# naver-ai/egtr

Measured on AMD Instinct MI355X. Metric: images/sec end-to-end SGG, 600x1000 input, N=200 queries, higher is better.
Workload: dtype f32; 1 GPU; VG inference: ResNet-50, N=200, 6 enc/6 dec, 150 classes, 50 predicates, 600x1000, bs=1/GPU fp32 (BASELINE configs[1]); hip_graph=True, gemm_tuning=True, miopen_find=True, parallelism=replicas x1 (independent images, no collective)

## Files before the change

### egtr_amd/csrc/rel_head.hip

```cpp
#include <hip/hip_runtime.h>
#include <stdint.h>

#include "common.h"
#include "xs_format.h"

namespace {

typedef float f32x16 __attribute__((ext_vector_type(16)));

__device__ __forceinline__ f32x16 mfma32(float a, float b, f32x16 c) {
  return __builtin_amdgcn_mfma_f32_32x32x2f32(a, b, c, 0, 0, 0);
}

constexpr int kHd = 256;
constexpr int kH1Stride = 260;

typedef float f32x4v __attribute__((ext_vector_type(4)));

template <int OFF>
__device__ __forceinline__ f32x4v gload_b128(const float4* p) {
  f32x4v v;
  asm volatile("global_load_dwordx4 %0, %1, off offset:%2" : "=&v"(v) : "v"(p), "n"(OFF));
  return v;
}
// ... 471 lines not shown
  float* dst = rel_logits + (size_t)p0 * R;
  for (int pp = 0; pp < npair; ++pp) {
    const int tb = s_tb[pp];
    for (int r = lane; r < R; r += 64) {
      float v = s_out[pp * kStride + r] + b3r[r];
      if (tb >= 0) v += triplet[tb + r];
      dst[(size_t)pp * R + r] = v;
    }
  }
}

constexpr int kHp = 264;

typedef float f32x2v __attribute__((ext_vector_type(2)));
using xs::pack_hi16;
using xs::Split3;

__device__ __forceinline__ f32x4v gload_b128_s(unsigned voff, const void* sbase) {
  f32x4v v;
  asm volatile("global_load_dwordx4 %0, %1, %2" : "=&v"(v) : "v"(voff), "s"(sbase));
  return v;
}
__device__ __forceinline__ f32x4v gload_b128_s1k(unsigned voff, const void* sbase) {
  f32x4v v;
  asm volatile("global_load_dwordx4 %0, %1, %2 offset:1024" : "=&v"(v) : "v"(voff), "s"(sbase));
  return v;
}
__device__ __forceinline__ f32x4v gload_b128_s2k(unsigned voff, const void* sbase) {
  f32x4v v;
  asm volatile("global_load_dwordx4 %0, %1, %2 offset:2048" : "=&v"(v) : "v"(voff), "s"(sbase));
  return v;
}

template <int PRE>
struct PrefetchX6 {
  template <int I>
  static __device__ __forceinline__ void issue(f32x4v (&wq)[PRE][3], unsigned voff, const char* wtile) {
    wq[I][0] = gload_b128_s(voff, wtile + I * 3072);
    wq[I][1] = gload_b128_s1k(voff, wtile + I * 3072);
    wq[I][2] = gload_b128_s2k(voff, wtile + I * 3072);
    if constexpr (I + 1 < PRE) issue<I + 1>(wq, voff, wtile);
  }
  template <int S>
  static __device__ __forceinline__ void run(f32x4v (&wq)[PRE][3], unsigned voff, const char* wtile,
                                             const __bf16* hrow, f32x16& acc_m, f32x16& acc_c) {
    constexpr int newer = 3 * ((15 - S) < (PRE - 1) ? (15 - S) : (PRE - 1));
    vm_wait<newer>(wq[S % PRE][0]);
    vm_wait<newer>(wq[S % PRE][1]);
    vm_wait<newer>(wq[S % PRE][2]);
    const bf16x8 whi = __builtin_bit_cast(bf16x8, wq[S % PRE][0]);
    const bf16x8 wmid = __builtin_bit_cast(bf16x8, wq[S % PRE][1]);
    const bf16x8 wlo = __builtin_bit_cast(bf16x8, wq[S % PRE][2]);
    const bf16x8 hhi = *reinterpret_cast<const bf16x8*>(hrow + 16 * S);
    const bf16x8 hmid = *reinterpret_cast<const bf16x8*>(hrow + 32 * kHp + 16 * S);
    const bf16x8 hlo = *reinterpret_cast<const bf16x8*>(hrow + 64 * kHp + 16 * S);
    acc_c = mfma_bf16(whi, hlo, acc_c);
    acc_m = mfma_bf16(whi, hhi, acc_m);
    acc_c = mfma_bf16(wlo, hhi, acc_c);
    acc_c = mfma_bf16(wmid, hmid, acc_c);
    acc_c = mfma_bf16(whi, hmid, acc_c);
    acc_c = mfma_bf16(wmid, hhi, acc_c);
    if constexpr (S + PRE < 16) {
      wq[S % PRE][0] = gload_b128_s(voff, wtile + (S + PRE) * 3072);
      wq[S % PRE][1] = gload_b128_s1k(voff, wtile + (S + PRE) * 3072);
      wq[S % PRE][2] = gload_b128_s2k(voff, wtile + (S + PRE) * 3072);
    }
    if constexpr (S + 1 < 16) run<S + 1>(wq, voff, wtile, hrow, acc_m, acc_c);
  }
};

template <int PRE>
struct PrefetchX1 {
  template <int I>
  static __device__ __forceinline__ void issue(f32x4v (&wq)[PRE][1], unsigned voff, const char* wtile) {
    wq[I][0] = gload_b128_s(voff, wtile + I * 1024);
    if constexpr (I + 1 < PRE) issue<I + 1>(wq, voff, wtile);
  }
  template <int S>
  static __device__ __forceinline__ void run(f32x4v (&wq)[PRE][1], unsigned voff, const char* wtile,
                                             const __bf16* hrow, f32x16& acc) {
    constexpr int newer = (15 - S) < (PRE - 1) ? (15 - S) : (PRE - 1);
    vm_wait<newer>(wq[S % PRE][0]);
    const bf16x8 w = __builtin_bit_cast(bf16x8, wq[S % PRE][0]);
    const bf16x8 h = *reinterpret_cast<const bf16x8*>(hrow + 16 * S);
    acc = mfma_bf16(w, h, acc);
    if constexpr (S + PRE < 16) wq[S % PRE][0] = gload_b128_s(voff, wtile + (S + PRE) * 1024);
    if constexpr (S + 1 < 16) run<S + 1>(wq, voff, wtile, hrow, acc);
  }
};

template <int T, int OT, bool SAVE = false, int TERMS = 6>
__global__ __launch_bounds__(64 * kRhWaves) __attribute__((amdgpu_waves_per_eu(2, 2))) void rel_head_fwd_x6(
    const float* __restrict__ gate_q, const float* __restrict__ gate_k, const float* __restrict__ uq,
    const float* __restrict__ uk, const float* __restrict__ b1, const unsigned short* __restrict__ w2xr,
    const float* __restrict__ b2r, const unsigned short* __restrict__ w3xr, const float* __restrict__ b3r,
    const unsigned short* __restrict__ w2xc, const float* __restrict__ b2c, const float* __restrict__ w3c,
    const float* __restrict__ b3c, const float* __restrict__ triplet, const int64_t* __restrict__ node_cls, int B,
    int N, int R, int C1, float* __restrict__ rel_logits, float* __restrict__ conn_logits,
    float* __restrict__ gate_mean, int apply_sigmoid, float* __restrict__ h1_save, float* __restrict__ h2_save) {
  static_assert(TERMS == 6 || TERMS == 1, "six exact cross terms or one product of rounded operands");
  constexpr int kPieces = TERMS == 6 ? 3 : 1;
  constexpr int kStride = 32 * OT + 1;
  static_assert(kRhWaves * 32 * kStride * 4 <= kPieces * 32 * kHp * 2, "output tiles fit in the h1 buffer");
  __shared__ __attribute__((aligned(16))) __bf16 s_h[kPieces * 32 * kHp];
  float* const s_out = reinterpret_cast<float*>(s_h);
  __shared__ int s_tb[32];
  __shared__ long long s_pp[32];
  __shared__ float s_cacc[kRhWaves][32];
  constexpr int kH2Pitch = 36;
  __shared__ __attribute__((aligned(16))) float s_h2[SAVE ? kRhWaves * 8 * kH2Pitch : 4];
  const int lane = threadIdx.x & 63, pi = lane & 31, hf = lane >> 5;
  const int wv = __builtin_amdgcn_readfirstlane(threadIdx.x >> 6);
  const int mlp = blockIdx.y;
  const long long total = (long long)B * N * N;
  const int tj = (N + 3) >> 2, ti = (N + 7) >> 3;
  const int b = blockIdx.x / (ti * tj);
  const int trem = blockIdx.x - b * ti * tj;
  const int i0 = (trem / tj) * 8, j0 = (trem - (trem / tj) * tj) * 4;
  const int i_raw = i0 + (pi >> 2), j_raw = j0 + (pi & 3);
  const bool valid = i_raw < N && j_raw < N;
  const int i = i_raw < N ? i_raw : N - 1, j = j_raw < N ? j_raw : N - 1;
  const long long p = ((long long)b * N + i) * N + j;
  const size_t qi = (size_t)b * N + i, kj = (size_t)b * N + j;

  if (SAVE && wv == 0 && hf == 0) s_pp[pi] = valid ? p : -1;
  float g[T];
#pragma unroll
  for (int t = 0; t < T; ++t) {
    const float x = gate_q[qi * T + t] + gate_k[kj * T + t];
    g[t] = 1.f / (1.f + expf(-x));
  }
  if (gate_mean != nullptr && mlp == 0 && wv == 0) {
#pragma unroll
    for (int t = 0; t < T; ++t) {
      float v = (valid && hf == 0) ? g[t] : 0.f;
#pragma unroll
      for (int o = 1; o < 64; o <<= 1) v += __shfl_xor(v, o);
      if (lane == 0) unsafeAtomicAdd(gate_mean + t, v / (float)total);
    }
  }

  {
    const int krow_l = (int)kj;
    const float4 bias4 = reinterpret_cast<const float4*>(b1 + mlp * kHd)[lane];
    const float4* uq4 = reinterpret_cast<const float4*>(uq) + mlp * (kHd / 4) + lane;
    const float4* uk4 = reinterpret_cast<const float4*>(uk) + mlp * (kHd / 4) + lane;
    constexpr int ROW4 = 2 * kHd / 4;
    float4 kk[4][T];
#pragma unroll
    for (int jj = 0; jj < 4; ++jj) {
      const int kr = __builtin_amdgcn_readlane(krow_l, jj);
      const float4* pk = uk4 + (size_t)kr * T * ROW4;
#pragma unroll
      for (int t = 0; t < T; ++t) kk[jj][t] = pk[t * ROW4];
    }
    auto qrow_of = [&](int ii) { return b * N + (i0 + ii < N ? i0 + ii : N - 1); };
    const int ii0 = wv * (8 / kRhWaves);
    float4 ua[2][T];
    {
      const float4* pq = uq4 + (size_t)qrow_of(ii0) * T * ROW4;
#pragma unroll
      for (int t = 0; t < T; ++t) ua[0][t] = pq[t * ROW4];
    }
#pragma unroll
    for (int iu = 0; iu < 8 / kRhWaves; ++iu) {
      const int ii = ii0 + iu;
      if (iu + 1 < 8 / kRhWaves) {
        const float4* pq = uq4 + (size_t)qrow_of(ii + 1) * T * ROW4;
#pragma unroll
        for (int t = 0; t < T; ++t) ua[(iu + 1) & 1][t] = pq[t * ROW4];
      }
#pragma unroll
      for (int jj = 0; jj < 4; ++jj) {
        const int pp = ii * 4 + jj;
        f32x2v a01 = {bias4.x, bias4.y}, a23 = {bias4.z, bias4.w};
#pragma unroll
        for (int t = 0; t < T; ++t) {
          const float4 a = ua[iu & 1][t];
          const float4 c = kk[jj][t];
          const float gt = __int_as_float(__builtin_amdgcn_readlane(__float_as_int(g[t]), pp));
          const f32x2v gg = {gt, gt};
          const f32x2v u01 = {a.x + c.x, a.y + c.y}, u23 = {a.z + c.z, a.w + c.w};
          a01 = gg * u01 + a01;
          a23 = gg * u23 + a23;
        }
        if (SAVE && i0 + ii < N && j0 + jj < N)
          reinterpret_cast<float4*>(h1_save + ((size_t)mlp * total +
                                               (size_t)(((long long)b * N + i0 + ii) * N + j0 + jj)) * kHd)[lane] =
              make_float4(egtr_relu(a01.x), egtr_relu(a01.y), egtr_relu(a23.x), egtr_relu(a23.y));
        if constexpr (TERMS == 1) {
          *reinterpret_cast<uint2*>(s_h + pp * kHp + 4 * lane) =
              make_uint2(xs::cvt_pk_bf16_rne(egtr_relu(a01.x), egtr_relu(a01.y)),
                         xs::cvt_pk_bf16_rne(egtr_relu(a23.x), egtr_relu(a23.y)));
        } else {
          const Split3 sx = xs::split3_fast(egtr_relu(a01.x)), sy = xs::split3_fast(egtr_relu(a01.y)),
                       sz = xs::split3_fast(egtr_relu(a23.x)), sw = xs::split3_fast(egtr_relu(a23.y));
          __bf16* hp = s_h + pp * kHp + 4 * lane;
          *reinterpret_cast<uint2*>(hp) = make_uint2(pack_hi16(sx.hi, sy.hi), pack_hi16(sz.hi, sw.hi));
          *reinterpret_cast<uint2*>(hp + 32 * kHp) = make_uint2(pack_hi16(sx.mid, sy.mid), pack_hi16(sz.mid, sw.mid));
          *reinterpret_cast<uint2*>(hp + 64 * kHp) = make_uint2(pack_hi16(sx.lo, sy.lo), pack_hi16(sz.lo, sw.lo));
        }
      }
    }
    __syncthreads();
  }

  const char* w2x = reinterpret_cast<const char*>(mlp ? w2xc : w2xr);
  const float* b2 = mlp ? b2c : b2r;
  f32x16 racc[OT];
#pragma unroll
  for (int ot = 0; ot < OT; ++ot)
#pragma unroll
    for (int r = 0; r < 16; ++r) racc[ot][r] = 0.f;
  float cacc = 0.f;
  const unsigned voff = (unsigned)lane * 16u;
  const __bf16* hrow = s_h + pi * kHp + 8 * hf;

  constexpr int kNtPerWave = kHd / 32 / kRhWaves;
#pragma unroll 1
  for (int nt = wv * kNtPerWave; nt < (wv + 1) * kNtPerWave; ++nt) {
    f32x16 acc, accc;
#pragma unroll
    for (int r = 0; r < 16; ++r) accc[r] = 0.f;
#pragma unroll
    for (int rq = 0; rq < 4; ++rq) {
      const float4 bb = *reinterpret_cast<const float4*>(b2 + nt * 32 + 8 * rq + 4 * hf);
      acc[4 * rq + 0] = bb.x; acc[4 * rq + 1] = bb.y; acc[4 * rq + 2] = bb.z; acc[4 * rq + 3] = bb.w;
    }
    constexpr int kFrag = kPieces * 1024;
    const char* wtile = w2x + (size_t)nt * (16 * kFrag);
    constexpr int kPre = 4;
    f32x4v wq[kPre][kPieces];
    f32x4v w3q[2 * OT][kPieces];
    if (mlp == 0) {
      const char* w3t = reinterpret_cast<const char*>(w3xr) + (size_t)nt * (2 * OT * kFrag);
#pragma unroll
      for (int f = 0; f < 2 * OT; ++f) {
        w3q[f][0] = gload_b128_s(voff, w3t + f * kFrag);
        if constexpr (TERMS == 6) {
          w3q[f][1] = gload_b128_s1k(voff, w3t + f * kFrag);
          w3q[f][2] = gload_b128_s2k(voff, w3t + f * kFrag);
        }
      }
    }
    if constexpr (TERMS == 1) {
      PrefetchX1<kPre>::template issue<0>(wq, voff, wtile);
      PrefetchX1<kPre>::template run<0>(wq, voff, wtile, hrow, acc);
#pragma unroll
      for (int r = 0; r < 16; ++r) acc[r] = egtr_relu(acc[r]);
    } else {
      PrefetchX6<kPre>::template issue<0>(wq, voff, wtile);
      PrefetchX6<kPre>::template run<0>(wq, voff, wtile, hrow, acc, accc);
#pragma unroll
      for (int r = 0; r < 16; ++r) acc[r] = egtr_relu(acc[r] + accc[r]);
    }
    if (SAVE) {
      float* stg = s_h2 + wv * (8 * kH2Pitch);
#pragma unroll
      for (int i = 0; i < 4; ++i) {
        if ((pi >> 3) == i) {
#pragma unroll
          for (int rq = 0; rq < 4; ++rq)
            *reinterpret_cast<float4*>(stg + (pi & 7) * kH2Pitch + 8 * rq + 4 * hf) =
                make_float4(acc[4 * rq + 0], acc[4 * rq + 1], acc[4 * rq + 2], acc[4 * rq + 3]);
        }
        __builtin_amdgcn_fence(__ATOMIC_RELEASE, "wavefront");
        __builtin_amdgcn_wave_barrier();
        __builtin_amdgcn_fence(__ATOMIC_ACQUIRE, "wavefront");
        const int pr = lane >> 3, ch = lane & 7;
        const float4 v = *reinterpret_cast<const float4*>(stg + pr * kH2Pitch + 4 * ch);
        const long long po = s_pp[8 * i + pr];
        if (po >= 0) *reinterpret_cast<float4*>(h2_save + ((size_t)mlp * total + (size_t)po) * kHd + nt * 32 + 4 * ch) = v;
        __builtin_amdgcn_fence(__ATOMIC_RELEASE, "wavefront");
        __builtin_amdgcn_wave_barrier();
        __builtin_amdgcn_fence(__ATOMIC_ACQUIRE, "wavefront");
      }
    }
    if (mlp == 0) {
#pragma unroll
      for (int f = 0; f < 2 * OT; ++f) {
        if constexpr (TERMS == 1) asm volatile("" : "+v"(w3q[f][0]));
        else asm volatile("" : "+v"(w3q[f][0]), "+v"(w3q[f][1]), "+v"(w3q[f][2]));
      }
#pragma unroll
      for (int kb = 0; kb < 2; ++kb) {
// ... 12 lines not shown
          Split3 sp[8];
#pragma unroll
          for (int e = 0; e < 8; ++e) sp[e] = xs::split3_fast(acc[8 * kb + e]);
          phi = make_uint4(pack_hi16(sp[0].hi, sp[1].hi), pack_hi16(sp[2].hi, sp[3].hi), pack_hi16(sp[4].hi, sp[5].hi),
                           pack_hi16(sp[6].hi, sp[7].hi));
          pmid = make_uint4(pack_hi16(sp[0].mid, sp[1].mid), pack_hi16(sp[2].mid, sp[3].mid),
                            pack_hi16(sp[4].mid, sp[5].mid), pack_hi16(sp[6].mid, sp[7].mid));
          plo = make_uint4(pack_hi16(sp[0].lo, sp[1].lo), pack_hi16(sp[2].lo, sp[3].lo), pack_hi16(sp[4].lo, sp[5].lo),
                           pack_hi16(sp[6].lo, sp[7].lo));
        }
        const bf16x8 hhi = __builtin_bit_cast(bf16x8, phi), hmid = __builtin_bit_cast(bf16x8, pmid),
                     hlo = __builtin_bit_cast(bf16x8, plo);
#pragma unroll
        for (int ot = 0; ot < OT; ++ot) {
          const bf16x8 whi = __builtin_bit_cast(bf16x8, w3q[kb * OT + ot][0]);
          const bf16x8 wmid = __builtin_bit_cast(bf16x8, w3q[kb * OT + ot][1]);
          const bf16x8 wlo = __builtin_bit_cast(bf16x8, w3q[kb * OT + ot][2]);
          racc[ot] = mfma_bf16(whi, hlo, racc[ot]);
          racc[ot] = mfma_bf16(wlo, hhi, racc[ot]);
          racc[ot] = mfma_bf16(wmid, hmid, racc[ot]);
          racc[ot] = mfma_bf16(whi, hmid, racc[ot]);
          racc[ot] = mfma_bf16(wmid, hhi, racc[ot]);
          racc[ot] = mfma_bf16(whi, hhi, racc[ot]);
        }
        }
      }
    } else {
#pragma unroll
      for (int rq = 0; rq < 4; ++rq) {
        const float4 w = *reinterpret_cast<const float4*>(w3c + nt * 32 + 8 * rq + 4 * hf);
        cacc += w.x * acc[4 * rq + 0] + w.y * acc[4 * rq + 1] + w.z * acc[4 * rq + 2] + w.w * acc[4 * rq + 3];
      }
    }
  }

  if (mlp == 1) {
    cacc += __shfl_xor(cacc, 32);
    if (hf == 0) s_cacc[wv][pi] = cacc;
    __syncthreads();
    if (wv == 0 && valid && hf == 0) {
      float v = s_cacc[0][pi];
#pragma unroll
      for (int w = 1; w < kRhWaves; ++w) v += s_cacc[w][pi];
      v += b3c[0];
      conn_logits[p] = apply_sigmoid ? 1.f / (1.f + expf(-v)) : v;
    }
    return;
  }
  __syncthreads();
  float* const my_out = s_out + wv * 32 * kStride;
#pragma unroll
  for (int ot = 0; ot < OT; ++ot)
#pragma unroll
    for (int r = 0; r < 16; ++r) {
      const int ro = ot * 32 + (r & 3) + 8 * (r >> 2) + 4 * hf;
      my_out[pi * kStride + ro] = racc[ot][r];
    }
  if (wv == 0 && hf == 0) {
    int tb = -1;
    if (triplet != nullptr) tb = ((int)node_cls[qi] * C1 + (int)node_cls[kj]) * R;
    s_tb[pi] = tb;
    s_pp[pi] = valid ? p : -1;
  }
  __syncthreads();
  for (int pp = wv; pp < 32; pp += kRhWaves) {
    const long long po = s_pp[pp];
    if (po < 0) continue;
    const int tb = s_tb[pp];
    float* dst = rel_logits + (size_t)po * R;
    for (int r = lane; r < R; r += 64) {
      float v = s_out[pp * kStride + r];
#pragma unroll
      for (int w = 1; w < kRhWaves; ++w) v += s_out[(w * 32 + pp) * kStride + r];
      v += b3r[r];
      if (tb >= 0) v += triplet[tb + r];
      dst[r] = apply_sigmoid ? 1.f / (1.f + expf(-v)) : v;
    }
  }
}

template <int T>
int launch_T(hipStream_t st, int R, dim3 grid, const float* gate_q, const float* gate_k, const float* uq,
             const float* uk, const float* b1, const float* w2r, const float* b2r, const float* w3r,
             const float* b3r, const float* w2c, const float* b2c, const float* w3c, const float* b3c,
             const float* triplet, const int64_t* node_cls, int B, int N, int C1, float* rel, float* conn,
             float* gate_mean, float* h1_save, float* h2_save) {
  if (R <= 32)
    hipLaunchKernelGGL((rel_head_fwd_f32<T, 1>), grid, dim3(64 * kRhWaves), 0, st, gate_q, gate_k, uq, uk, b1, w2r, b2r, w3r,
                       b3r, w2c, b2c, w3c, b3c, triplet, node_cls, B, N, R, C1, rel, conn, gate_mean, h1_save,
                       h2_save);
  else
    hipLaunchKernelGGL((rel_head_fwd_f32<T, 2>), grid, dim3(64 * kRhWaves), 0, st, gate_q, gate_k, uq, uk, b1, w2r, b2r, w3r,
                       b3r, w2c, b2c, w3c, b3c, triplet, node_cls, B, N, R, C1, rel, conn, gate_mean, h1_save,
                       h2_save);
  return 0;
}

template <int T, bool KPASS>
__global__ __launch_bounds__(256) void rel_head_bwd_pairs_f32(
    const float* __restrict__ dh1, const float* __restrict__ gate_q, const float* __restrict__ gate_k,
    const float* __restrict__ utab , int B, int N,
    float* __restrict__ dutab , float* __restrict__ dz ,
    float* __restrict__ dgate_k ) {
  __shared__ float s_g[256 * T];
  __shared__ __attribute__((aligned(16))) float s_red[4 * T * 512];
  __shared__ float s_dk[4 * T];
  const int tid = threadIdx.x, lane = tid & 63, wave = tid >> 6;
  const int b = blockIdx.x / N, f = blockIdx.x - b * N;
  const size_t total = (size_t)B * N * N;
  const float* gfix = (KPASS ? gate_k : gate_q) + ((size_t)b * N + f) * T;
  const float* gvar = (KPASS ? gate_q : gate_k) + (size_t)b * N * T;
// ... 191 lines not shown
    if (num_rel <= 32)                                                                                               \
      hipLaunchKernelGGL((rel_head_fwd_bf16w<TT, 1>), grid, dim3(64), 0, st, gate_q, gate_k, uq, uk, b1, w2r, b2r, w3r, \
                         b3r, w2c, b2c, w3c, b3c, triplet_dist, node_cls, batch, num_query, num_rel, num_cls_plus1,  \
                         rel_logits, conn_logits, gate_mean);                                                        \
    else                                                                                                             \
      hipLaunchKernelGGL((rel_head_fwd_bf16w<TT, 2>), grid, dim3(64), 0, st, gate_q, gate_k, uq, uk, b1, w2r, b2r, w3r, \
                         b3r, w2c, b2c, w3c, b3c, triplet_dist, node_cls, batch, num_query, num_rel, num_cls_plus1,  \
                         rel_logits, conn_logits, gate_mean);                                                        \
    break;
  switch (num_slots) {
    EGTR_TB(1) EGTR_TB(2) EGTR_TB(3) EGTR_TB(4) EGTR_TB(5) EGTR_TB(6) EGTR_TB(7) EGTR_TB(8) EGTR_TB(9) EGTR_TB(10)
    default: return EGTR_E_UNSUPPORTED;
  }
#undef EGTR_TB
  return egtr_check_launch();
}


extern "C" int egtr_rel_head_forward_bf16x6_f32(egtr_stream_t stream, const float* gate_q, const float* gate_k,
                                                const float* uq, const float* uk, const float* b1,
                                                const uint16_t* w2x_rel, const float* b2r, const uint16_t* w3x_rel,
                                                const float* b3r, const uint16_t* w2x_conn, const float* b2c,
                                                const float* w3c, const float* b3c, const float* triplet_dist,
                                                const int64_t* node_cls, int batch, int num_query, int num_slots,
                                                int hidden, int num_rel, int num_cls_plus1, float* rel_logits,
                                                float* conn_logits, float* gate_mean, int apply_sigmoid) {
  if (!gate_q || !gate_k || !uq || !uk || !b1 || !w2x_rel || !b2r || !w3x_rel || !b3r || !w2x_conn || !b2c || !w3c ||
      !b3c || !rel_logits || !conn_logits)
    return EGTR_E_ARG;
  if (triplet_dist != nullptr && node_cls == nullptr) return EGTR_E_ARG;
  if (batch <= 0 || num_query <= 0 || num_slots <= 0 || num_rel <= 0) return EGTR_E_ARG;
  if (hidden != kHd || num_rel > 64 || num_slots > 9) return EGTR_E_UNSUPPORTED;
  hipStream_t st = static_cast<hipStream_t>(stream);
  const long long tiles = (long long)batch * ((num_query + 7) / 8) * ((num_query + 3) / 4);
  if (tiles >= (1ll << 31)) return EGTR_E_UNSUPPORTED;
  const dim3 grid((unsigned)tiles, 2);
#define EGTR_TX(TT)                                                                                                  \
  case TT:                                                                                                           \
    if (num_rel <= 32)                                                                                               \
      hipLaunchKernelGGL((rel_head_fwd_x6<TT, 1>), grid, dim3(64 * kRhWaves), 0, st, gate_q, gate_k, uq, uk, b1,     \
                         w2x_rel, b2r, w3x_rel, b3r, w2x_conn, b2c, w3c, b3c, triplet_dist, node_cls, batch,         \
                         num_query, num_rel, num_cls_plus1, rel_logits, conn_logits, gate_mean, apply_sigmoid,       \
                         (float*)nullptr, (float*)nullptr);                                                          \
    else                                                                                                             \
      hipLaunchKernelGGL((rel_head_fwd_x6<TT, 2>), grid, dim3(64 * kRhWaves), 0, st, gate_q, gate_k, uq, uk, b1,     \
                         w2x_rel, b2r, w3x_rel, b3r, w2x_conn, b2c, w3c, b3c, triplet_dist, node_cls, batch,         \
                         num_query, num_rel, num_cls_plus1, rel_logits, conn_logits, gate_mean, apply_sigmoid,       \
                         (float*)nullptr, (float*)nullptr);                                                          \
    break;
  switch (num_slots) {
    EGTR_TX(1) EGTR_TX(2) EGTR_TX(3) EGTR_TX(4) EGTR_TX(5) EGTR_TX(6) EGTR_TX(7) EGTR_TX(8) EGTR_TX(9)
    default: return EGTR_E_UNSUPPORTED;
  }
#undef EGTR_TX
  return egtr_check_launch();
}

extern "C" int egtr_rel_head_forward_bf16x6_save_f32(egtr_stream_t stream, const float* gate_q, const float* gate_k,
                                                     const float* uq, const float* uk, const float* b1,
                                                     const uint16_t* w2x_rel, const float* b2r, const uint16_t* w3x_rel,
                                                     const float* b3r, const uint16_t* w2x_conn, const float* b2c,
                                                     const float* w3c, const float* b3c, const float* triplet_dist,
                                                     const int64_t* node_cls, int batch, int num_query, int num_slots,
                                                     int hidden, int num_rel, int num_cls_plus1, float* rel_logits,
                                                     float* conn_logits, float* gate_mean, float* h1_save,
                                                     float* h2_save) {
  if (!gate_q || !gate_k || !uq || !uk || !b1 || !w2x_rel || !b2r || !w3x_rel || !b3r || !w2x_conn || !b2c || !w3c ||
      !b3c || !rel_logits || !conn_logits || !h1_save || !h2_save)
    return EGTR_E_ARG;
  if (triplet_dist != nullptr && node_cls == nullptr) return EGTR_E_ARG;
  if (batch <= 0 || num_query <= 0 || num_rel <= 0) return EGTR_E_ARG;
  if (hidden != kHd || num_rel > 64 || (num_slots != 4 && num_slots != 7)) return EGTR_E_UNSUPPORTED;
  hipStream_t st = static_cast<hipStream_t>(stream);
  const long long tiles = (long long)batch * ((num_query + 7) / 8) * ((num_query + 3) / 4);
  if (tiles >= (1ll << 31)) return EGTR_E_UNSUPPORTED;
  const dim3 grid((unsigned)tiles, 2);
#define EGTR_TXS(TT, OTT)                                                                                            \
  hipLaunchKernelGGL((rel_head_fwd_x6<TT, OTT, true>), grid, dim3(64 * kRhWaves), 0, st, gate_q, gate_k, uq, uk, b1,  \
                     w2x_rel, b2r, w3x_rel, b3r, w2x_conn, b2c, w3c, b3c, triplet_dist, node_cls, batch, num_query,   \
                     num_rel, num_cls_plus1, rel_logits, conn_logits, gate_mean, 0, h1_save, h2_save)
  if (num_slots == 4) {
    if (num_rel <= 32) EGTR_TXS(4, 1); else EGTR_TXS(4, 2);
  } else {
    if (num_rel <= 32) EGTR_TXS(7, 1); else EGTR_TXS(7, 2);
  }
#undef EGTR_TXS
// ... 65 lines not shown
        d[0] = (unsigned short)(xs::bf16_rne_bits(w) >> 16);
      } else {
        const xs::Split3 sp = xs::split3_rne(w);
        d[0] = (unsigned short)(sp.hi >> 16);
        d[512] = (unsigned short)(sp.mid >> 16);
        d[1024] = (unsigned short)(sp.lo >> 16);
      }
    }
  }
}
}

extern "C" int egtr_rel_head_streams_f32(egtr_stream_t stream, const float* w2_rel, const float* w2_conn,
                                         const float* w3_rel, int hidden, int num_rel, uint16_t* w2x_rel,
                                         uint16_t* w2x_conn, uint16_t* w3x_rel) {
  if (!w2_rel || !w2_conn || !w3_rel || !w2x_rel || !w2x_conn || !w3x_rel || num_rel <= 0) return EGTR_E_ARG;
  if (hidden != kHd || num_rel > 64) return EGTR_E_UNSUPPORTED;
  const int OT = num_rel <= 32 ? 1 : 2;
  hipLaunchKernelGGL(rel_head_streams_f32<3>, dim3(256), dim3(256), 0, static_cast<hipStream_t>(stream), w2_rel, w2_conn,
                     w3_rel, num_rel, OT, w2x_rel, w2x_conn, w3x_rel);
  return egtr_check_launch();
}

extern "C" int egtr_rel_head_streams_bf16r_f32(egtr_stream_t stream, const float* w2_rel, const float* w2_conn,
                                               const float* w3_rel, int hidden, int num_rel, uint16_t* w2x_rel,
                                               uint16_t* w2x_conn, uint16_t* w3x_rel) {
  if (!w2_rel || !w2_conn || !w3_rel || !w2x_rel || !w2x_conn || !w3x_rel || num_rel <= 0) return EGTR_E_ARG;
  if (hidden != kHd || num_rel > 64) return EGTR_E_UNSUPPORTED;
  const int OT = num_rel <= 32 ? 1 : 2;
  hipLaunchKernelGGL(rel_head_streams_f32<1>, dim3(256), dim3(256), 0, static_cast<hipStream_t>(stream), w2_rel, w2_conn,
                     w3_rel, num_rel, OT, w2x_rel, w2x_conn, w3x_rel);
  return egtr_check_launch();
}
```

### egtr_amd/kernels/heads.py

```python
import torch

from .. import _lib
from .._lib import _chk
from .linear import _split3_bf16

__all__ = ["rel_head_split_weights", "rel_head_streams", "relation_head_split_bf16", "relation_head_train_forward", "hungarian_match",
           "pack_detection_targets", "pack_relation_bits", "relation_loss_launch", "relation_loss_all_launch"]


def _rel_head_pieces(w, terms):
    if terms not in (1, 6):
        raise ValueError(f"terms must be 6 (split-bf16, fp32 accuracy) or 1 (operands rounded to bf16), got {terms!r}")
    return _split3_bf16(w) if terms == 6 else w.detach().float().to(torch.bfloat16).unsqueeze(0)


def rel_head_split_weights(w2r, w3r, w2c, terms=6):
    pieces = _rel_head_pieces(w2r, terms).shape[0]

    def w2x(w2):
        p = _rel_head_pieces(w2, terms).view(pieces, 8, 32, 16, 2, 8)
        p = p.permute(1, 3, 0, 4, 2, 5).contiguous()
        return p if terms == 6 else p.squeeze(2)

    R = w3r.shape[0]
    OT = 1 if R <= 32 else 2
    w3p = torch.zeros(32 * OT, w3r.shape[1], dtype=torch.float32, device=w3r.device)
    w3p[:R] = w3r.detach().float()
    q = _rel_head_pieces(w3p, terms).view(pieces, OT, 32, w3r.shape[1])
    dev = w3r.device
    nt = torch.arange(8, device=dev).view(8, 1, 1, 1)
    kb = torch.arange(2, device=dev).view(1, 2, 1, 1)
    hf = torch.arange(2, device=dev).view(1, 1, 2, 1)
    e = torch.arange(8, device=dev).view(1, 1, 1, 8)
    nidx = 32 * nt + 16 * kb + (e & 3) + 8 * (e >> 2) + 4 * hf
    g = q[:, :, :, nidx]
    w3x = g.permute(3, 4, 1, 0, 5, 2, 6).contiguous()
    if terms == 1:
        w3x = w3x.squeeze(3)
    return w2x(w2r), w3x, w2x(w2c)

# ... 49 lines not shown
                b2c_.data_ptr(), w3c_.data_ptr(), b3c_.data_ptr(), _lib.ptr(triplet_dist),
                _lib.ptr(node_cls if triplet_dist is not None else None), B, N, T, Hd, R, c1, rel.data_ptr(),
                conn.data_ptr(), _lib.ptr(gm), h1s.data_ptr(), h2s.data_ptr())
    return rel, conn, gm, h1s, h2s


def relation_head_split_bf16(gate_q, gate_k, uq, uk, b1, w2x_rel, b2r, w3x_rel, b3r, w2x_conn, b2c, w3c, b3c,
                             num_rel, triplet_dist=None, node_cls=None, want_gate_mean=False, sigmoid=False):
    B, N, T = gate_q.shape
    dev = gate_q.device
    f32 = [_chk(t.detach().contiguous(), n, torch.float32)
           for t, n in ((gate_q, "gate_q"), (gate_k, "gate_k"), (uq, "uq"), (uk, "uk"), (b1, "b1"), (b2r, "b2r"),
                        (b3r, "b3r"), (b2c, "b2c"), (w3c, "w3c"), (b3c, "b3c"))]
    gq, gk, uq_, uk_, b1_, b2r_, b3r_, b2c_, w3c_, b3c_ = f32
    R = int(num_rel)
    OT = 1 if R <= 32 else 2
    for t, n, shape in ((w2x_rel, "w2x_rel", (8, 16, 3, 2, 32, 8)), (w2x_conn, "w2x_conn", (8, 16, 3, 2, 32, 8)),
                        (w3x_rel, "w3x_rel", (8, 2, OT, 3, 2, 32, 8))):
        _chk(t, n, torch.bfloat16)
        if tuple(t.shape) != shape:
            raise RuntimeError(f"{n} must have shape {shape}, got {tuple(t.shape)}")
    rel = torch.empty(B, N, N, R, dtype=torch.float32, device=dev)
    conn = torch.empty(B, N, N, dtype=torch.float32, device=dev)
    gm = torch.zeros(T, dtype=torch.float32, device=dev) if want_gate_mean else None
    td = None
    c1 = 0
    if triplet_dist is not None:
        td = _chk(triplet_dist.detach().contiguous(), "triplet_dist", torch.float32)
        _chk(node_cls, "node_cls", torch.int64)
        c1 = td.shape[0]
    _lib.launch("egtr_rel_head_forward_bf16x6_f32", gq.data_ptr(), gk.data_ptr(), uq_.data_ptr(), uk_.data_ptr(),
                b1_.data_ptr(), w2x_rel.data_ptr(), b2r_.data_ptr(), w3x_rel.data_ptr(), b3r_.data_ptr(), w2x_conn.data_ptr(),
                b2c_.data_ptr(), w3c_.data_ptr(), b3c_.data_ptr(), _lib.ptr(td), _lib.ptr(node_cls if td is not None else None),
                B, N, T, 256, R, c1, rel.data_ptr(), conn.data_ptr(), _lib.ptr(gm), 1 if sigmoid else 0)
    return rel, conn.unsqueeze(-1), gm


@torch.no_grad()
def hungarian_match(logits, pred_boxes, targets, class_cost, bbox_cost, giou_cost, cost_min=None,
                    inverse_sigmoid_smoothing=None, cost_in=None, want_cost=False, want_status=False):
    lib = _lib.lib()
    if cost_in is not None:
        B = len(cost_in)
        N = cost_in[0].shape[0]
        dev = cost_in[0].device
        sizes = [int(c.shape[1]) for c in cost_in]
        cin = torch.cat([_chk(c.contiguous(), "cost_in", torch.float32).reshape(-1) for c in cost_in]) \
            if sum(sizes) else torch.zeros(1, device=dev)
        K = 0
        lg = bx = ti = tb = None
    else:
        B, N, K = logits.shape
        dev = logits.device
        sizes = [int(t["boxes"].shape[0]) for t in targets]
        lg = _chk(logits.detach().contiguous(), "logits", torch.float32)
        bx = _chk(pred_boxes.detach().contiguous(), "pred_boxes", torch.float32)
        ti = torch.cat([t["class_labels"] for t in targets]).to(device=dev, dtype=torch.int64).contiguous()
        tb = torch.cat([t["boxes"] for t in targets]).to(device=dev, dtype=torch.float32).contiguous()
        cin = None
    n_out = [min(N, t) for t in sizes]
    offs = [0]
    for t in sizes:
        offs.append(offs[-1] + t)
    ooffs = [0]
    for t in n_out:
        ooffs.append(ooffs[-1] + t)
    meta = torch.tensor(offs + ooffs, dtype=torch.int32).to(dev, non_blocking=True)
# ... 86 lines not shown
```

Baseline: 401.1 images/sec.

## Add 64-pair tile relation head kernel reusing weight fragments across two pair groups

Adds a new relation-head forward kernel that processes 8x8 query pairs per block (64 pairs) instead of 8x4. Each weight fragment loaded from global memory now feeds MFMAs for two 32-pair groups, halving weight traffic per pair. The layer-2 hidden dimension is split into two halves with layer-1 recomputed per half, and layer-3 weights are prefetched during the layer-2 tail. It is enabled by default through a Python flag, with the old kernel kept behind a bit in the sigmoid argument. Optional compile-time timing instrumentation is also added. The cost is more accumulator registers per wave, which limits occupancy.

```diff
diff --git a/egtr_amd/csrc/rel_head.hip b/egtr_amd/csrc/rel_head.hip
--- a/egtr_amd/csrc/rel_head.hip
+++ b/egtr_amd/csrc/rel_head.hip
@@ -527,6 +527,39 @@
   return v;
 }
 
+#ifdef EGTR_REL_HEAD_TIMING
+constexpr int kRhRecWg = 256, kRhRecN = 16;
+__device__ unsigned g_rel_head_rec[2][kRhRecWg][kRhRecN];
+#define RH_T(v)                                         \
+  do {                                                  \
+    __builtin_amdgcn_sched_barrier(0);                  \
+    (v) = (unsigned)__builtin_amdgcn_s_memtime();       \
+    __builtin_amdgcn_sched_barrier(0);                  \
+  } while (0)
+#if EGTR_REL_HEAD_TIMING > 1
+#define RH_TW_PARAM , unsigned& tw_
+#define RH_TW_ARG , tw_
+#define RH_TW0(a) a; RH_T(tw0_)
+#define RH_TW1(sum, a)        \
+  do {                        \
+    unsigned b_;              \
+    RH_T(b_);                 \
+    (sum) += b_ - (a);        \
+  } while (0)
+#else
+#define RH_TW_PARAM
+#define RH_TW_ARG
+#define RH_TW0(a) do { } while (0)
+#define RH_TW1(sum, a) do { } while (0)
+#endif
+#else
+#define RH_T(v) do { } while (0)
+#define RH_TW_PARAM
+#define RH_TW_ARG
+#define RH_TW0(a) do { } while (0)
+#define RH_TW1(sum, a) do { } while (0)
+#endif
+
 template <int PRE>
 struct PrefetchX6 {
   template <int I>
@@ -538,11 +571,13 @@
   }
   template <int S>
   static __device__ __forceinline__ void run(f32x4v (&wq)[PRE][3], unsigned voff, const char* wtile,
-                                             const __bf16* hrow, f32x16& acc_m, f32x16& acc_c) {
+                                             const __bf16* hrow, f32x16& acc_m, f32x16& acc_c RH_TW_PARAM) {
     constexpr int newer = 3 * ((15 - S) < (PRE - 1) ? (15 - S) : (PRE - 1));
+    RH_TW0(unsigned tw0_);
     vm_wait<newer>(wq[S % PRE][0]);
     vm_wait<newer>(wq[S % PRE][1]);
     vm_wait<newer>(wq[S % PRE][2]);
+    RH_TW1(tw_, tw0_);
     const bf16x8 whi = __builtin_bit_cast(bf16x8, wq[S % PRE][0]);
     const bf16x8 wmid = __builtin_bit_cast(bf16x8, wq[S % PRE][1]);
     const bf16x8 wlo = __builtin_bit_cast(bf16x8, wq[S % PRE][2]);
@@ -560,7 +595,7 @@
       wq[S % PRE][1] = gload_b128_s1k(voff, wtile + (S + PRE) * 3072);
       wq[S % PRE][2] = gload_b128_s2k(voff, wtile + (S + PRE) * 3072);
     }
-    if constexpr (S + 1 < 16) run<S + 1>(wq, voff, wtile, hrow, acc_m, acc_c);
+    if constexpr (S + 1 < 16) run<S + 1>(wq, voff, wtile, hrow, acc_m, acc_c RH_TW_ARG);
   }
 };
 
@@ -618,6 +653,10 @@
   const long long p = ((long long)b * N + i) * N + j;
   const size_t qi = (size_t)b * N + i, kj = (size_t)b * N + j;
 
+#ifdef EGTR_REL_HEAD_TIMING
+  unsigned tk0, tg, tl1, ta, tb_, tc, tloop[4] = {0, 0, 0, 0}, tl3[4] = {0, 0, 0, 0}, tpre = 0, tw_ = 0;
+  RH_T(tk0);
+#endif
   if (SAVE && wv == 0 && hf == 0) s_pp[pi] = valid ? p : -1;
   float g[T];
 #pragma unroll
@@ -635,6 +674,7 @@
     }
   }
 
+  RH_T(tg);
   {
     const int krow_l = (int)kj;
     const float4 bias4 = reinterpret_cast<const float4*>(b1 + mlp * kHd)[lane];
@@ -699,6 +739,7 @@
     }
     __syncthreads();
   }
+  RH_T(tl1);
 
   const char* w2x = reinterpret_cast<const char*>(mlp ? w2xc : w2xr);
   const float* b2 = mlp ? b2c : b2r;
@@ -714,6 +755,7 @@
   constexpr int kNtPerWave = kHd / 32 / kRhWaves;
 #pragma unroll 1
   for (int nt = wv * kNtPerWave; nt < (wv + 1) * kNtPerWave; ++nt) {
+    RH_T(ta);
     f32x16 acc, accc;
 #pragma unroll
     for (int r = 0; r < 16; ++r) accc[r] = 0.f;
@@ -745,7 +787,9 @@
       for (int r = 0; r < 16; ++r) acc[r] = egtr_relu(acc[r]);
     } else {
       PrefetchX6<kPre>::template issue<0>(wq, voff, wtile);
-      PrefetchX6<kPre>::template run<0>(wq, voff, wtile, hrow, acc, accc);
+      RH_T(tb_);
+      PrefetchX6<kPre>::template run<0>(wq, voff, wtile, hrow, acc, accc RH_TW_ARG);
+      RH_T(tc);
 #pragma unroll
       for (int r = 0; r < 16; ++r) acc[r] = egtr_relu(acc[r] + accc[r]);
     }
@@ -824,7 +868,43 @@
         cacc += w.x * acc[4 * rq + 0] + w.y * acc[4 * rq + 1] + w.z * acc[4 * rq + 2] + w.w * acc[4 * rq + 3];
       }
     }
-  }
+#ifdef EGTR_REL_HEAD_TIMING
+    if constexpr (TERMS == 6) {
+      unsigned td;
+      RH_T(td);
+      const int q = nt - wv * kNtPerWave;
+      tpre += tb_ - ta;
+#pragma unroll
+      for (int k = 0; k < 4; ++k)
+        if (q == k) {
+          tloop[k] = tc - tb_;
+          tl3[k] = td - tc;
+        }
+    }
+#endif
+  }
+#ifdef EGTR_REL_HEAD_TIMING
+  auto rh_record = [&]() {
+    if constexpr (!SAVE && TERMS == 6) {
+      asm volatile("s_waitcnt vmcnt(0)" ::: "memory");
+      unsigned tk1;
+      RH_T(tk1);
+      if (threadIdx.x == 0 && (blockIdx.x & 15) == 0 && (blockIdx.x >> 4) < kRhRecWg) {
+        unsigned* rec = g_rel_head_rec[mlp][blockIdx.x >> 4];
+        rec[0] = tg - tk0;
+        rec[1] = tl1 - tg;
+        for (int k = 0; k < 4; ++k) {
+          rec[2 + k] = tloop[k];
+          rec[6 + k] = tl3[k];
+        }
+        rec[10] = tpre;
+        rec[11] = tk1 - tc - tl3[3];
+        rec[12] = tk1 - tk0;
+        rec[13] = tw_;
+      }
+    }
+  };
+#endif
 
   if (mlp == 1) {
     cacc += __shfl_xor(cacc, 32);
@@ -837,6 +917,9 @@
       v += b3c[0];
       conn_logits[p] = apply_sigmoid ? 1.f / (1.f + expf(-v)) : v;
     }
+#ifdef EGTR_REL_HEAD_TIMING
+    rh_record();
+#endif
     return;
   }
   __syncthreads();
@@ -869,6 +952,384 @@
       dst[r] = apply_sigmoid ? 1.f / (1.f + expf(-v)) : v;
     }
   }
+#ifdef EGTR_REL_HEAD_TIMING
+  rh_record();
+#endif
+}
+
+constexpr int kHp64 = 136;
+constexpr int kP64Waves = 4;
+constexpr int kFragX6 = 3072;
+constexpr int kP64TwoRows = 7;
+
+__device__ __forceinline__ void gload_frag(f32x4v (&w)[3], unsigned voff, const char* p) {
+  w[0] = gload_b128_s(voff, p);
+  w[1] = gload_b128_s1k(voff, p);
+  w[2] = gload_b128_s2k(voff, p);
+}
+template <int NEWER>
+__device__ __forceinline__ void vm_wait_frag(f32x4v (&w)[3]) {
+  vm_wait<NEWER>(w[0]);
+  vm_wait<NEWER>(w[1]);
+  vm_wait<NEWER>(w[2]);
+}
+
+template <int PRE, int OT>
+struct PrefetchP64 {
+  static constexpr int kW3 = 4 * OT;
+  static_assert(16 % PRE == 0 && PRE <= kW3, "slot = index mod PRE; the first W3 requests are the refills of the second half");
+  static __device__ __forceinline__ const char* frag(const char* wbase, int F, int H) {
+    return wbase + (F & 1) * (16 * kFragX6) + (8 * H + (F >> 1)) * kFragX6;
+  }
+  template <int H, int I = 0>
+  static __device__ __forceinline__ void issue(f32x4v (&wq)[PRE][3], unsigned voff, const char* wbase) {
+    gload_frag(wq[I], voff, frag(wbase, I, H));
+    if constexpr (I + 1 < PRE) issue<H, I + 1>(wq, voff, wbase);
+  }
+  template <int H, int F = 0>
+  static __device__ __forceinline__ void run(f32x4v (&wq)[PRE][3], unsigned voff, const char* wbase, const char* w3base,
+                                             bool rel, const __bf16* hrow, bf16x8 (&hh)[2][3], f32x16 (&acc)[2][2],
+                                             f32x16 (&accc)[2][2] RH_TW_PARAM) {
+    constexpr int s = F >> 1, a = F & 1;
+    constexpr int newer = (15 - F) < (PRE - 1) ? (15 - F) : (PRE - 1);
+    RH_TW0(unsigned tw0_);
+    if constexpr (H == 1 && F + PRE > 16) {
+      constexpr int newer_rel = (15 + kW3 - F) < (PRE - 1) ? (15 + kW3 - F) : (PRE - 1);
+      if (rel) vm_wait_frag<3 * newer_rel>(wq[F % PRE]);
+      else vm_wait_frag<3 * newer>(wq[F % PRE]);
+    } else {
+      vm_wait_frag<3 * newer>(wq[F % PRE]);
+    }
+    RH_TW1(tw_, tw0_);
+    const bf16x8 whi = __builtin_bit_cast(bf16x8, wq[F % PRE][0]);
+    const bf16x8 wmid = __builtin_bit_cast(bf16x8, wq[F % PRE][1]);
+    const bf16x8 wlo = __builtin_bit_cast(bf16x8, wq[F % PRE][2]);
+    if constexpr (a == 0) {
+#pragma unroll
+      for (int P = 0; P < 2; ++P)
+#pragma unroll
+        for (int pc = 0; pc < 3; ++pc)
+          hh[P][pc] = *reinterpret_cast<const bf16x8*>(hrow + (pc * 64 + P * 32) * kHp64 + 16 * s);
+    }
+    accc[a][0] = mfma_bf16(whi, hh[0][2], accc[a][0]);
+    accc[a][1] = mfma_bf16(whi, hh[1][2], accc[a][1]);
+    acc[a][0] = mfma_bf16(whi, hh[0][0], acc[a][0]);
+    acc[a][1] = mfma_bf16(whi, hh[1][0], acc[a][1]);
+    accc[a][0] = mfma_bf16(wlo, hh[0][0], accc[a][0]);
+    accc[a][1] = mfma_bf16(wlo, hh[1][0], accc[a][1]);
+    accc[a][0] = mfma_bf16(wmid, hh[0][1], accc[a][0]);
+    accc[a][1] = mfma_bf16(wmid, hh[1][1], accc[a][1]);
+    accc[a][0] = mfma_bf16(whi, hh[0][1], accc[a][0]);
+    accc[a][1] = mfma_bf16(whi, hh[1][1], accc[a][1]);
+    accc[a][0] = mfma_bf16(wmid, hh[0][0], accc[a][0]);
+    accc[a][1] = mfma_bf16(wmid, hh[1][0], accc[a][1]);
+    if constexpr (F + PRE < 16) {
+      gload_frag(wq[F % PRE], voff, frag(wbase, F + PRE, H));
+    } else if constexpr (H == 1 && F + PRE - 16 < kW3) {
+      if (rel) gload_frag(wq[F % PRE], voff, w3base + (F + PRE - 16) * kFragX6);
+    }
+    if constexpr (F + 1 < 16) run<H, F + 1>(wq, voff, wbase, w3base, rel, hrow, hh, acc, accc RH_TW_ARG);
+  }
+  template <int J = 0>
+  static __device__ __forceinline__ void layer3(f32x4v (&wq)[PRE][3], unsigned voff, const char* w3base, bf16x8 (&hh)[2][3],
+                                                const f32x16 (&acc)[2][2], f32x16 (&racc)[2][OT]) {
+    constexpr int a = J / (2 * OT), kb = (J / OT) & 1, ot = J % OT;
+    if constexpr (ot == 0) {
+#pragma unroll
+      for (int P = 0; P < 2; ++P) {
+        Split3 sp[8];
+#pragma unroll
+        for (int e = 0; e < 8; ++e) sp[e] = xs::split3_fast(acc[a][P][8 * kb + e]);
+        hh[P][0] = __builtin_bit_cast(bf16x8, make_uint4(pack_hi16(sp[0].hi, sp[1].hi), pack_hi16(sp[2].hi, sp[3].hi),
+                                                         pack_hi16(sp[4].hi, sp[5].hi), pack_hi16(sp[6].hi, sp[7].hi)));
+        hh[P][1] = __builtin_bit_cast(bf16x8, make_uint4(pack_hi16(sp[0].mid, sp[1].mid), pack_hi16(sp[2].mid, sp[3].mid),
+                                                         pack_hi16(sp[4].mid, sp[5].mid), pack_hi16(sp[6].mid, sp[7].mid)));
+        hh[P][2] = __builtin_bit_cast(bf16x8, make_uint4(pack_hi16(sp[0].lo, sp[1].lo), pack_hi16(sp[2].lo, sp[3].lo),
+                                                         pack_hi16(sp[4].lo, sp[5].lo), pack_hi16(sp[6].lo, sp[7].lo)));
+      }
+    }
+    constexpr int newer = (kW3 - 1 - J) < (PRE - 1) ? (kW3 - 1 - J) : (PRE - 1);
+    vm_wait_frag<3 * newer>(wq[J % PRE]);
+    const bf16x8 whi = __builtin_bit_cast(bf16x8, wq[J % PRE][0]);
+    const bf16x8 wmid = __builtin_bit_cast(bf16x8, wq[J % PRE][1]);
+    const bf16x8 wlo = __builtin_bit_cast(bf16x8, wq[J % PRE][2]);
+    racc[0][ot] = mfma_bf16(whi, hh[0][2], racc[0][ot]);
+    racc[1][ot] = mfma_bf16(whi, hh[1][2], racc[1][ot]);
+    racc[0][ot] = mfma_bf16(wlo, hh[0][0], racc[0][ot]);
+    racc[1][ot] = mfma_bf16(wlo, hh[1][0], racc[1][ot]);
+    racc[0][ot] = mfma_bf16(wmid, hh[0][1], racc[0][ot]);
+    racc[1][ot] = mfma_bf16(wmid, hh[1][1], racc[1][ot]);
+    racc[0][ot] = mfma_bf16(whi, hh[0][1], racc[0][ot]);
+    racc[1][ot] = mfma_bf16(whi, hh[1][1], racc[1][ot]);
+    racc[0][ot] = mfma_bf16(wmid, hh[0][0], racc[0][ot]);
+    racc[1][ot] = mfma_bf16(wmid, hh[1][0], racc[1][ot]);
+    racc[0][ot] = mfma_bf16(whi, hh[0][0], racc[0][ot]);
+    racc[1][ot] = mfma_bf16(whi, hh[1][0], racc[1][ot]);
+    if constexpr (J + PRE < kW3) gload_frag(wq[J % PRE], voff, w3base + (J + PRE) * kFragX6);
+    if constexpr (J + 1 < kW3) layer3<J + 1>(wq, voff, w3base, hh, acc, racc);
+  }
+};
+
+template <int T, int OT>
+__global__ __launch_bounds__(64 * kP64Waves) __attribute__((amdgpu_waves_per_eu(2, 2))) void rel_head_fwd_x6p64(
+    const float* __restrict__ gate_q, const float* __restrict__ gate_k, const float* __restrict__ uq,
+    const float* __restrict__ uk, const float* __restrict__ b1, const unsigned short* __restrict__ w2xr,
+    const float* __restrict__ b2r, const unsigned short* __restrict__ w3xr, const float* __restrict__ b3r,
+    const unsigned short* __restrict__ w2xc, const float* __restrict__ b2c, const float* __restrict__ w3c,
+    const float* __restrict__ b3c, const float* __restrict__ triplet, const int64_t* __restrict__ node_cls, int B,
+    int N, int R, int C1, float* __restrict__ rel_logits, float* __restrict__ conn_logits,
+    float* __restrict__ gate_mean, int apply_sigmoid) {
+  constexpr int kStride = 32 * OT + 1;
+  static_assert(kP64Waves * 32 * kStride * 4 <= 3 * 64 * kHp64 * 2, "the output tiles of one pair tile fit in the h1 buffer");
+  __shared__ __attribute__((aligned(16))) __bf16 s_h[3 * 64 * kHp64];
+  float* const s_out = reinterpret_cast<float*>(s_h);
+  __shared__ int s_tb[64];
+  __shared__ long long s_pp[64];
+  __shared__ float s_cacc[kP64Waves][64];
+  const int lane = threadIdx.x & 63, pi = lane & 31, hf = lane >> 5;
+  const int wv = __builtin_amdgcn_readfirstlane(threadIdx.x >> 6);
+  const int mlp = blockIdx.y;
+  const bool rel = mlp == 0;
+  const long long total = (long long)B * N * N;
+  const int t8 = (N + 7) >> 3;
+  const int b = blockIdx.x / (t8 * t8);
+  const int trem = blockIdx.x - b * t8 * t8;
+  const int i0 = (trem / t8) * 8, j0 = (trem - (trem / t8) * t8) * 8;
+  const int i_raw = i0 + (pi >> 2), j_raw = j0 + 4 * hf + (pi & 3);
+  const bool valid = i_raw < N && j_raw < N;
+  const int i = i_raw < N ? i_raw : N - 1, j = j_raw < N ? j_raw : N - 1;
+  const long long p = ((long long)b * N + i) * N + j;
+  const size_t qi = (size_t)b * N + i, kj = (size_t)b * N + j;
+#ifdef EGTR_REL_HEAD_TIMING
+  unsigned tk0, tg, ts[6], tw_ = 0;
+  RH_T(tk0);
+#endif
+
+  if (gate_mean != nullptr && rel && wv == 0) {
+#pragma unroll
+    for (int t = 0; t < T; ++t) {
+      const float x = gate_q[qi * T + t] + gate_k[kj * T + t];
+      float v = valid ? 1.f / (1.f + expf(-x)) : 0.f;
+#pragma unroll
+      for (int o = 1; o < 64; o <<= 1) v += __shfl_xor(v, o);
+      if (lane == 0) unsafeAtomicAdd(gate_mean + t, v / (float)total);
+    }
+  }
+  const size_t krow = (size_t)b * N + (j0 + 2 * wv + hf < N ? j0 + 2 * wv + hf : N - 1);
+  auto qrow_of = [&](int ii) { return (size_t)b * N + (i0 + ii < N ? i0 + ii : N - 1); };
+  float g[T];
+  {
+    const size_t gq = qrow_of(pi & 7);
+#pragma unroll
+    for (int t = 0; t < T; ++t) {
+      const float x = gate_q[gq * T + t] + gate_k[krow * T + t];
+      g[t] = 1.f / (1.f + expf(-x));
+    }
+  }
+  RH_T(tg);
+
+  constexpr int ROW4 = 2 * kHd / 4;
+  auto layer1 = [&](int H) {
+    const int c4 = 32 * H + pi;
+    const float4 bias4 = reinterpret_cast<const float4*>(b1 + mlp * kHd)[c4];
+    const float4* uq4 = reinterpret_cast<const float4*>(uq) + mlp * (kHd / 4) + c4;
+    const float4* uk4 = reinterpret_cast<const float4*>(uk) + mlp * (kHd / 4) + c4;
+    float4 kk[T];
+    {
+      const float4* pk = uk4 + krow * T * ROW4;
+#pragma unroll
+      for (int t = 0; t < T; ++t) kk[t] = pk[t * ROW4];
+    }
+    __bf16* const hcol = s_h + (32 * (wv >> 1) + 2 * (wv & 1) + hf) * kHp64 + 4 * pi;
+    auto load_row = [&](float4 (&u)[T], int ii) {
+      const float4* pq = uq4 + qrow_of(ii) * T * ROW4;
+#pragma unroll
+      for (int t = 0; t < T; ++t) u[t] = pq[t * ROW4];
+    };
+    auto row = [&](const float4 (&u)[T], int ii) {
+      f32x2v a01 = {bias4.x, bias4.y}, a23 = {bias4.z, bias4.w};
+#pragma unroll
+      for (int t = 0; t < T; ++t) {
+        const float4 a = u[t];
+        const float4 c = kk[t];
+        const float gt = __shfl(g[t], 32 * hf + ii);
+        const f32x2v gg = {gt, gt};
+        const f32x2v u01 = {a.x + c.x, a.y + c.y}, u23 = {a.z + c.z, a.w + c.w};
+        a01 = gg * u01 + a01;
+        a23 = gg * u23 + a23;
+      }
+      const Split3 sx = xs::split3_fast(egtr_relu(a01.x)), sy = xs::split3_fast(egtr_relu(a01.y)),
+                   sz = xs::split3_fast(egtr_relu(a23.x)), sw = xs::split3_fast(egtr_relu(a23.y));
+      __bf16* hp = hcol + 4 * ii * kHp64;
+      *reinterpret_cast<uint2*>(hp) = make_uint2(pack_hi16(sx.hi, sy.hi), pack_hi16(sz.hi, sw.hi));
+      *reinterpret_cast<uint2*>(hp + 64 * kHp64) = make_uint2(pack_hi16(sx.mid, sy.mid), pack_hi16(sz.mid, sw.mid));
+      *reinterpret_cast<uint2*>(hp + 128 * kHp64) = make_uint2(pack_hi16(sx.lo, sy.lo), pack_hi16(sz.lo, sw.lo));
+    };
+    if constexpr (T <= kP64TwoRows) {
+      float4 ua[2][T];
+      load_row(ua[0], 0);
+#pragma unroll 1
+      for (int ii = 0; ii < 8; ii += 2) {
+        load_row(ua[1], ii + 1);
+        row(ua[0], ii);
+        if (ii + 2 < 8) load_row(ua[0], ii + 2);
+        row(ua[1], ii + 1);
+      }
+    } else {
+      float4 ua[T];
+#pragma unroll 1
+      for (int ii = 0; ii < 8; ++ii) {
+        load_row(ua, ii);
+        row(ua, ii);
+      }
+    }
+  };
+
+  const char* const wbase = reinterpret_cast<const char*>(rel ? w2xr : w2xc) + (size_t)(2 * wv) * (16 * kFragX6);
+  const char* const w3base = reinterpret_cast<const char*>(w3xr) + (size_t)(2 * wv) * (2 * OT * kFragX6);
+  const float* b2 = rel ? b2r : b2c;
+  const unsigned voff = (unsigned)lane * 16u;
+  const __bf16* hrow = s_h + pi * kHp64 + 8 * hf;
+  constexpr int kPre = 4;
+  using Q = PrefetchP64<kPre, OT>;
+  f32x4v wq[kPre][3];
+  bf16x8 hh[2][3];
+  f32x16 acc[2][2], accc[2][2];
+
+  layer1(0);
+  Q::template issue<0>(wq, voff, wbase);
+#pragma unroll
+  for (int a = 0; a < 2; ++a) {
+#pragma unroll
+    for (int rq = 0; rq < 4; ++rq) {
+      const float4 bb = *reinterpret_cast<const float4*>(b2 + (2 * wv + a) * 32 + 8 * rq + 4 * hf);
+#pragma unroll
+      for (int P = 0; P < 2; ++P) {
+        acc[a][P][4 * rq + 0] = bb.x; acc[a][P][4 * rq + 1] = bb.y; acc[a][P][4 * rq + 2] = bb.z; acc[a][P][4 * rq + 3] = bb.w;
+      }
+    }
+#pragma unroll
+    for (int P = 0; P < 2; ++P)
+#pragma unroll
+      for (int r = 0; r < 16; ++r) accc[a][P][r] = 0.f;
+  }
+  __syncthreads();
+  RH_T(ts[0]);
+  Q::template run<0>(wq, voff, wbase, w3base, rel, hrow, hh, acc, accc RH_TW_ARG);
+  RH_T(ts[1]);
+  __syncthreads();
+  RH_T(ts[2]);
+  layer1(1);
+  Q::template issue<1>(wq, voff, wbase);
+  __syncthreads();
+  RH_T(ts[3]);
+  Q::template run<1>(wq, voff, wbase, w3base, rel, hrow, hh, acc, accc RH_TW_ARG);
+  RH_T(ts[4]);
+#pragma unroll
+  for (int a = 0; a < 2; ++a)
+#pragma unroll
+    for (int P = 0; P < 2; ++P)
+#pragma unroll
+      for (int r = 0; r < 16; ++r) acc[a][P][r] = egtr_relu(acc[a][P][r] + accc[a][P][r]);
+
+#ifdef EGTR_REL_HEAD_TIMING
+  auto rh_record = [&]() {
+    asm volatile("s_waitcnt vmcnt(0)" ::: "memory");
+    unsigned tk1;
+    RH_T(tk1);
+    if (threadIdx.x == 0 && (blockIdx.x & 15) == 0 && (blockIdx.x >> 4) < kRhRecWg) {
+      unsigned* rec = g_rel_head_rec[mlp][blockIdx.x >> 4];
+      rec[0] = tg - tk0;
+      rec[1] = ts[0] - tg;
+      rec[2] = ts[1] - ts[0];
+      rec[3] = ts[2] - ts[1];
+      rec[4] = ts[3] - ts[2];
+      rec[5] = ts[4] - ts[3];
+      rec[6] = ts[5] - ts[4];
+      rec[11] = tk1 - ts[5];
+      rec[12] = tk1 - tk0;
+      rec[13] = tw_;
+    }
+  };
+#endif
+
+  if (!rel) {
+    float cacc[2] = {0.f, 0.f};
+#pragma unroll
+    for (int a = 0; a < 2; ++a)
+#pragma unroll
+      for (int rq = 0; rq < 4; ++rq) {
+        const float4 w = *reinterpret_cast<const float4*>(w3c + (2 * wv + a) * 32 + 8 * rq + 4 * hf);
+#pragma unroll
+        for (int P = 0; P < 2; ++P)
+          cacc[P] += w.x * acc[a][P][4 * rq + 0] + w.y * acc[a][P][4 * rq + 1] + w.z * acc[a][P][4 * rq + 2] +
+                     w.w * acc[a][P][4 * rq + 3];
+      }
+#pragma unroll
+    for (int P = 0; P < 2; ++P) {
+      cacc[P] += __shfl_xor(cacc[P], 32);
+      if (hf == 0) s_cacc[wv][32 * P + pi] = cacc[P];
+    }
+    RH_T(ts[5]);
+    __syncthreads();
+    if (wv == 0 && valid) {
+      float v = s_cacc[0][lane];
+#pragma unroll
+      for (int w = 1; w < kP64Waves; ++w) v += s_cacc[w][lane];
+      v += b3c[0];
+      conn_logits[p] = apply_sigmoid ? 1.f / (1.f + expf(-v)) : v;
+    }
+#ifdef EGTR_REL_HEAD_TIMING
+    rh_record();
+#endif
+    return;
+  }
+
+  f32x16 racc[2][OT];
+#pragma unroll
+  for (int P = 0; P < 2; ++P)
+#pragma unroll
+    for (int ot = 0; ot < OT; ++ot)
+#pragma unroll
+      for (int r = 0; r < 16; ++r) racc[P][ot][r] = 0.f;
+  Q::template layer3<0>(wq, voff, w3base, hh, acc, racc);
+  RH_T(ts[5]);
+  if (wv == 0) {
+    int tb = -1;
+    if (triplet != nullptr) tb = ((int)node_cls[qi] * C1 + (int)node_cls[kj]) * R;
+    s_tb[lane] = tb;
+    s_pp[lane] = valid ? p : -1;
+  }
+  float* const my_out = s_out + wv * 32 * kStride;
+#pragma unroll
+  for (int P = 0; P < 2; ++P) {
+    __syncthreads();
+#pragma unroll
+    for (int ot = 0; ot < OT; ++ot)
+#pragma unroll
+      for (int r = 0; r < 16; ++r) {
+        const int ro = ot * 32 + (r & 3) + 8 * (r >> 2) + 4 * hf;
+        my_out[pi * kStride + ro] = racc[P][ot][r];
+      }
+    __syncthreads();
+    for (int pp = wv; pp < 32; pp += kP64Waves) {
+      const long long po = s_pp[32 * P + pp];
+      if (po < 0) continue;
+      const int tb = s_tb[32 * P + pp];
+      float* dst = rel_logits + (size_t)po * R;
+      for (int r = lane; r < R; r += 64) {
+        float v = s_out[pp * kStride + r];
+#pragma unroll
+        for (int w = 1; w < kP64Waves; ++w) v += s_out[(w * 32 + pp) * kStride + r];
+        v += b3r[r];
+        if (tb >= 0) v += triplet[tb + r];
+        dst[r] = apply_sigmoid ? 1.f / (1.f + expf(-v)) : v;
+      }
+    }
+  }
+#ifdef EGTR_REL_HEAD_TIMING
+  rh_record();
+#endif
 }
 
 template <int T>
@@ -1126,26 +1587,32 @@
   if (batch <= 0 || num_query <= 0 || num_slots <= 0 || num_rel <= 0) return EGTR_E_ARG;
   if (hidden != kHd || num_rel > 64 || num_slots > 9) return EGTR_E_UNSUPPORTED;
   hipStream_t st = static_cast<hipStream_t>(stream);
-  const long long tiles = (long long)batch * ((num_query + 7) / 8) * ((num_query + 3) / 4);
+  const bool p64 = (apply_sigmoid & 2) == 0;
+  const int sig = apply_sigmoid & 1;
+  const int tj = p64 ? (num_query + 7) / 8 : (num_query + 3) / 4;
+  const long long tiles = (long long)batch * ((num_query + 7) / 8) * tj;
   if (tiles >= (1ll << 31)) return EGTR_E_UNSUPPORTED;
   const dim3 grid((unsigned)tiles, 2);
-#define EGTR_TX(TT)                                                                                                  \
-  case TT:                                                                                                           \
-    if (num_rel <= 32)                                                                                               \
-      hipLaunchKernelGGL((rel_head_fwd_x6<TT, 1>), grid, dim3(64 * kRhWaves), 0, st, gate_q, gate_k, uq, uk, b1,     \
-                         w2x_rel, b2r, w3x_rel, b3r, w2x_conn, b2c, w3c, b3c, triplet_dist, node_cls, batch,         \
-                         num_query, num_rel, num_cls_plus1, rel_logits, conn_logits, gate_mean, apply_sigmoid,       \
-                         (float*)nullptr, (float*)nullptr);                                                          \
-    else                                                                                                             \
-      hipLaunchKernelGGL((rel_head_fwd_x6<TT, 2>), grid, dim3(64 * kRhWaves), 0, st, gate_q, gate_k, uq, uk, b1,     \
-                         w2x_rel, b2r, w3x_rel, b3r, w2x_conn, b2c, w3c, b3c, triplet_dist, node_cls, batch,         \
-                         num_query, num_rel, num_cls_plus1, rel_logits, conn_logits, gate_mean, apply_sigmoid,       \
-                         (float*)nullptr, (float*)nullptr);                                                          \
+#define EGTR_TXO(TT, OTT)                                                                                            \
+  if (p64)                                                                                                           \
+    hipLaunchKernelGGL((rel_head_fwd_x6p64<TT, OTT>), grid, dim3(64 * kP64Waves), 0, st, gate_q, gate_k, uq, uk, b1,  \
+                       w2x_rel, b2r, w3x_rel, b3r, w2x_conn, b2c, w3c, b3c, triplet_dist, node_cls, batch, num_query, \
+                       num_rel, num_cls_plus1, rel_logits, conn_logits, gate_mean, sig);                             \
+  else                                                                                                               \
+    hipLaunchKernelGGL((rel_head_fwd_x6<TT, OTT>), grid, dim3(64 * kRhWaves), 0, st, gate_q, gate_k, uq, uk, b1,     \
+                       w2x_rel, b2r, w3x_rel, b3r, w2x_conn, b2c, w3c, b3c, triplet_dist, node_cls, batch, num_query, \
+                       num_rel, num_cls_plus1, rel_logits, conn_logits, gate_mean, sig, (float*)nullptr,             \
+                       (float*)nullptr)
+#define EGTR_TX(TT)                        \
+  case TT:                                 \
+    if (num_rel <= 32) { EGTR_TXO(TT, 1); } \
+    else { EGTR_TXO(TT, 2); }               \
     break;
   switch (num_slots) {
     EGTR_TX(1) EGTR_TX(2) EGTR_TX(3) EGTR_TX(4) EGTR_TX(5) EGTR_TX(6) EGTR_TX(7) EGTR_TX(8) EGTR_TX(9)
     default: return EGTR_E_UNSUPPORTED;
   }
+#undef EGTR_TXO
 #undef EGTR_TX
   return egtr_check_launch();
 }
@@ -1277,3 +1744,11 @@
                      w3_rel, num_rel, OT, w2x_rel, w2x_conn, w3x_rel);
   return egtr_check_launch();
 }
+
+#ifdef EGTR_REL_HEAD_TIMING
+extern "C" int egtr_rel_head_stamps(unsigned* host_out) {
+  return hipMemcpyFromSymbol(host_out, HIP_SYMBOL(g_rel_head_rec), sizeof(unsigned) * 2 * kRhRecWg * kRhRecN) == hipSuccess
+             ? EGTR_OK
+             : EGTR_E_LAUNCH;
+}
+#endif
diff --git a/egtr_amd/kernels/heads.py b/egtr_amd/kernels/heads.py
--- a/egtr_amd/kernels/heads.py
+++ b/egtr_amd/kernels/heads.py
@@ -6,6 +6,9 @@
 
 __all__ = ["rel_head_split_weights", "rel_head_streams", "relation_head_split_bf16", "relation_head_train_forward", "hungarian_match",
            "pack_detection_targets", "pack_relation_bits", "relation_loss_launch", "relation_loss_all_launch"]
+
+
+REL_HEAD_PAIRS64 = True
 
 
 def _rel_head_pieces(w, terms):
@@ -121,7 +124,7 @@
     _lib.launch("egtr_rel_head_forward_bf16x6_f32", gq.data_ptr(), gk.data_ptr(), uq_.data_ptr(), uk_.data_ptr(),
                 b1_.data_ptr(), w2x_rel.data_ptr(), b2r_.data_ptr(), w3x_rel.data_ptr(), b3r_.data_ptr(), w2x_conn.data_ptr(),
                 b2c_.data_ptr(), w3c_.data_ptr(), b3c_.data_ptr(), _lib.ptr(td), _lib.ptr(node_cls if td is not None else None),
-                B, N, T, 256, R, c1, rel.data_ptr(), conn.data_ptr(), _lib.ptr(gm), 1 if sigmoid else 0)
+                B, N, T, 256, R, c1, rel.data_ptr(), conn.data_ptr(), _lib.ptr(gm), (1 if sigmoid else 0) | (0 if REL_HEAD_PAIRS64 else 2))
     return rel, conn.unsqueeze(-1), gm
 
 
```

Result: no change. 402.6 images/sec, median of 6 (+0.4%).
